# bcgsc/ntJoin

Hardware: AMD Instinct MI355X
Metric: Gbp/s minimizer-sketch+graph-build (k=32,w=1000) (higher is better)
Workload: dtype u64

## Files before the change

ntjoin_amd/csrc/graph.hip:

```cpp
#include <algorithm>
#include <cstdlib>
#include <cstring>
#include <system_error>
#include <thread>

#include "join_verdict.h"
#include "mxg_internal.h"
#include "scan_kernels.h"

namespace mxg {

static constexpr uint64_t HT_EMPTY = 0xFFFFFFFFFFFFFFFFull;
static constexpr uint32_t NONE32 = 0xFFFFFFFFu;

struct Slot {
    unsigned long long key;
    uint32_t nseen, ndup;
};

__device__ __forceinline__ uint32_t ht_slot(Slot *tab, uint32_t mask, uint32_t cap, uint64_t key)
{
    if (key == HT_EMPTY) return cap;
    uint32_t s = (uint32_t)((key * 0x9E3779B97F4A7C15ull) >> 32) & mask;
    while (true) {
        unsigned long long cur = tab[s].key;
        if (cur == key) return s;
        if (cur == HT_EMPTY) {
            unsigned long long old = atomicCAS(&tab[s].key, (unsigned long long)HT_EMPTY, (unsigned long long)key);
            if (old == HT_EMPTY || old == key) return s;
        }
        s = (s + 1) & mask;
    }
}

struct AsmSet {
    uint32_t n_asm;
    uint32_t full;
    uint32_t n[MXG_MAX_ASSEMBLIES];
    const uint32_t *n_ptr[MXG_MAX_ASSEMBLIES];
// ... 852 lines not shown
    const uint32_t rec = p.rec[i];
    p.vpos[v] = p.pos[i];
    p.vrec[v] = rec;
    if (p.ivid) p.ivid[i] = v;
    p.fv[r] = v;
    p.frec[r] = rec;
}

__global__ __launch_bounds__(256) void k_block_prefix(const uint32_t *__restrict__ cnt, const uint32_t *__restrict__ sup, uint32_t n,
                                                      uint32_t *__restrict__ out)
{
    __shared__ uint32_t sh[256];
    __shared__ uint32_t sh_before;
    const uint32_t e = blockIdx.x * 256u + threadIdx.x;
    const uint32_t c = e < n ? cnt[e] : 0u;
    if (threadIdx.x < 64) {
        const uint32_t bef = count_prefix(cnt, sup, blockIdx.x * 256u);
        if (threadIdx.x == 0) sh_before = bef;
    }
    __syncthreads();
    const uint32_t r = sh_before + block_exclusive_256(c, sh);
    if (e < n) out[e] = r;
}

struct VertexPjParams {
    AsmSet as;
    const uint32_t *pos[MXG_MAX_ASSEMBLIES], *rec[MXG_MAX_ASSEMBLIES];
    const uint32_t *cnt, *sup;
    uint64_t *n_shared;
    const uint64_t *mask0;
    const uint32_t *bpref0;
    uint64_t *vhash;
    uint32_t *vpos, *vrec, *fv, *frec;
    uint32_t nvs;
    uint32_t *ivid[MXG_MAX_ASSEMBLIES];
};

template <uint32_t U>
__global__ __launch_bounds__(256) void k_vertices_pj(const VertexPjParams p, uint32_t nb)
{
    __shared__ TailScan<U> ts;
    const uint32_t blk0 = blockIdx.x * U, lane = threadIdx.x & 63u, wv = threadIdx.x >> 6;
    TailAsm t[U];
    tail_asms<U>(p.as, blk0, nb, t);
    uint32_t ia[U], ii[U], vw[U], rec[U], pos[U];
    uint64_t hsh[U];
    bool in[U], f[U];
    {
        uint8_t fl[U];
#pragma unroll
        for (uint32_t u = 0; u < U; ++u) {
            const bool there = blk0 + u < nb;
            const uint32_t a = ia[u] = t[u].a, i = ii[u] = ((there ? blk0 + u : blk0) - t[u].b0) * 256u + threadIdx.x;
            in[u] = there && i < t[u].n;
            const uint32_t ic = in[u] ? i : 0u;
            fl[u] = p.as.flags[a][ic];
            vw[u] = p.as.slot[a][a ? ic : 0u];
            rec[u] = p.rec[a][ic];
            pos[u] = p.pos[a][ic];
            hsh[u] = p.as.hash[0][a ? 0u : ic];
        }
#pragma unroll
        for (uint32_t u = 0; u < U; ++u) f[u] = in[u] & ((fl[u] & MXG_MX_SHARED) != 0);
    }
    uint32_t v0[U];
#pragma unroll
// ... 16 lines not shown
            const uint64_t own = q == 0 ? mlo[g].x : q == 1 ? mlo[g].y : q == 2 ? mhi[g].x : mhi[g].y;
            v0[h + g] = bp[g] + (uint32_t)__popcll(own & ((1ull << (i0 & 63u)) - 1ull)) + (q > 0 ? (uint32_t)__popcll(mlo[g].x) : 0u) +
                        (q > 1 ? (uint32_t)__popcll(mlo[g].y) : 0u) + (q > 2 ? (uint32_t)__popcll(mhi[g].x) : 0u);
        }
        if (U > 2) __builtin_amdgcn_sched_barrier(0);
    }
    uint64_t bm[U];
#pragma unroll
    for (uint32_t u = 0; u < U; ++u) tail_ballot(ts, u, f[u], bm[u]);
    if (wv < U && blk0 + wv < nb) {
        const uint32_t blk_g = blk0 + wv, a = asm_of_block(p.as, blk_g);
        const uint32_t blk = blk_g - p.as.bstart[a], nblk = p.as.bstart[a + 1] - p.as.bstart[a];
        const uint32_t *cnt = p.cnt + p.as.bstart[a], *sup = p.sup + sup_start(p.as, a);
        const uint32_t bef = count_prefix(cnt, sup, blk);
        if (lane == 0) ts.before[wv] = bef;
        if (blk + 1 == nblk) {
            const uint32_t all = count_prefix(cnt, sup, nblk);
            if (lane == 0) p.n_shared[a] = all;
        }
    }
    __syncthreads();
#pragma unroll
    for (uint32_t u = 0; u < U; ++u) {
        if (!in[u]) continue;
        const uint32_t a = ia[u], i = ii[u];
        const uint32_t r = ts.before[u] + tail_rank(ts, u, bm[u]);
        const uint32_t v = a ? v0[u] : r;
        if (p.ivid[a]) p.ivid[a][i] = f[u] ? v : NONE32;
        if (!f[u]) continue;
        if (!a) p.vhash[v] = hsh[u];
        const size_t o = (size_t)a * p.nvs;
        p.vpos[o + v] = pos[u];
        p.vrec[o + v] = rec[u];
        p.fv[o + r] = v;
        p.frec[o + r] = rec[u];
    }
}

template <uint32_t U>
__global__ __launch_bounds__(256) void k_adjacency(const uint32_t *__restrict__ fv0, const uint32_t *__restrict__ frec0,
                                                   const uint64_t *__restrict__ nv_ptr, uint2 *__restrict__ adj0, uint32_t stride)
{
    const size_t o = (size_t)blockIdx.y * stride;
    const uint32_t *fv = fv0 + o, *frec = frec0 + o;
    uint32_t rc[U], rn[U], rp[U], vc[U], vn[U], vp[U];
#pragma unroll
    for (uint32_t u = 0; u < U; ++u) {
        const uint32_t r = (blockIdx.x * U + u) * 256u + threadIdx.x;
        rc[u] = rn[u] = rp[u] = vc[u] = vn[u] = vp[u] = 0;
        if (r < stride) {
            rc[u] = frec[r];
            vc[u] = fv[r];
            if (r + 1 < stride) {
                rn[u] = frec[r + 1];
                vn[u] = fv[r + 1];
            }
            if (r > 0) {
                rp[u] = frec[r - 1];
                vp[u] = fv[r - 1];
            }
        }
    }
    const uint32_t nv = (uint32_t)*nv_ptr;
#pragma unroll
    for (uint32_t u = 0; u < U; ++u) {
        const uint32_t r = (blockIdx.x * U + u) * 256u + threadIdx.x;
        if (r >= nv) continue;
        const uint32_t nx = (r + 1 < nv && rn[u] == rc[u]) ? vn[u] : NONE32;
        const uint32_t pv = (r > 0 && rp[u] == rc[u]) ? vp[u] : NONE32;
        adj0[o + vc[u]] = make_uint2(nx, pv);
    }
}

struct EdgeParams {
    const uint32_t *fv;
    const uint2 *adj;
    const uint64_t *nv_ptr;
    uint32_t nv, n_asm;
    uint8_t *eflag;
    uint32_t *bsum;
    uint32_t *bsuper;
    uint64_t *n_edges;
    uint64_t *host_ctl;
    uint32_t *eu, *ev, *esup;
    double *ew;
    double weights[MXG_MAX_ASSEMBLIES];
};

__device__ __forceinline__ uint32_t edge_mask(const EdgeParams &p, uint32_t u, uint32_t v)
{
    uint32_t m = 0;
    for (uint32_t b = 0; b < p.n_asm; ++b) {
        const uint2 q = p.adj[(size_t)b * p.nv + u];
        if (q.x == v || q.y == v) m |= 1u << b;
    }
    return m;
}

template <uint32_t U>
__global__ __launch_bounds__(256) void k_edge_flags(const EdgeParams p, uint32_t n_items)
{
    __shared__ TailScan<U> ts;
    const uint32_t blk0 = blockIdx.x * U, nblk = (n_items + 255u) / 256u, lane = threadIdx.x & 63u, wv = threadIdx.x >> 6;
    uint32_t uu[U], ia[U];
    bool live[U];
#pragma unroll
    for (uint32_t u = 0; u < U; ++u) {
        const uint32_t item = (blk0 + u) * 256u + threadIdx.x;
        uu[u] = p.fv[blk0 + u < nblk && item < n_items ? item : 0u];
// ... 56 lines not shown
    __shared__ TailScan<U> ts;
    const uint32_t blk0 = blockIdx.x * U, nblk = (n_items + 255u) / 256u, lane = threadIdx.x & 63u, wv = threadIdx.x >> 6;
    uint32_t fb[U], uu[U], v[U], m[U];
#pragma unroll
    for (uint32_t u = 0; u < U; ++u) {
        const uint32_t item = (blk0 + u) * 256u + threadIdx.x;
        const bool in = blk0 + u < nblk && item < n_items;
        fb[u] = p.eflag[in ? item : 0u];
        uu[u] = p.fv[in ? item : 0u];
        if (!in) fb[u] = 0;
    }
#pragma unroll
    for (uint32_t u = 0; u < U; ++u)
        v[u] = p.adj[fb[u] ? (size_t)(((blk0 + u) * 256u + threadIdx.x) / p.nv) * p.nv + uu[u] : (size_t)0].x;
    uint64_t bm[U];
#pragma unroll
    for (uint32_t u = 0; u < U; ++u) tail_ballot(ts, u, fb[u] != 0, bm[u]);
    if (wv < U && blk0 + wv < nblk) {
        const uint32_t bef = count_prefix(p.bsum, p.bsuper, blk0 + wv);
        if (lane == 0) ts.before[wv] = bef;
        if (blk0 + wv + 1 == nblk) {
            const uint32_t all = count_prefix(p.bsum, p.bsuper, nblk);
            if (lane == 0) {
                *p.n_edges = all;
                p.host_ctl[32] = all;
            }
            if (lane < p.n_asm) p.host_ctl[lane] = p.nv_ptr[lane];
        }
    }
#pragma unroll
    for (uint32_t u = 0; u < U; ++u) {
        m[u] = fb[u];
        if (fb[u] && p.n_asm > 8u) m[u] = edge_mask(p, uu[u], v[u]);
    }
    __syncthreads();
#pragma unroll
    for (uint32_t u = 0; u < U; ++u) {
        if (!fb[u]) continue;
        double wsum = 0.0;
        for (uint32_t b = 0; b < p.n_asm; ++b)
            if (m[u] & (1u << b)) wsum = wsum + p.weights[b];
        const uint32_t e = ts.before[u] + tail_rank(ts, u, bm[u]);
        p.eu[e] = uu[u];
        p.ev[e] = v[u];
        p.esup[e] = m[u];
        p.ew[e] = wsum;
    }
}

__global__ __launch_bounds__(256) void k_apply_msgs(const uint4 *__restrict__ msgs, uint64_t n, uint32_t stride, uint32_t *adj)
{
    const uint64_t i = (uint64_t)blockIdx.x * 256u + threadIdx.x;
    if (i >= n) return;
    const uint4 m = msgs[i];
    adj[((size_t)(m.x & 255u) * stride + m.y) * 2u + ((m.x >> 8) ? 1u : 0u)] = m.z;
}

__global__ __launch_bounds__(256) void k_iota_rows(uint32_t *a, uint32_t stride)
{
    const uint32_t i = blockIdx.x * 256u + threadIdx.x;
    if (i < stride) a[(size_t)blockIdx.y * stride + i] = i;
}

template <class T>
static int d2h(mxg_handle *h, std::vector<T> &dst, const void *src, size_t n)
{
// ... 51 lines not shown
    uint32_t pj_force_fail = 0;
    uint64_t *pj_mask0 = nullptr;
    uint32_t *pj_bpref0 = nullptr;
    AsmSet as_all;
    uint32_t n_fsup = 0, n_esup = 0;
    uint32_t *fsup = nullptr, *esup = nullptr, *cnt = nullptr;
    uint32_t *M = nullptr, *cursor = nullptr;
    uint4 *recs1 = nullptr, *recs2 = nullptr;
    PjSubCaps sc;
    size_t clear_words = 0;
};

static int plan_join(mxg_handle *h, int mode, const GraphBounds *gb, bool global_table, bool split, JoinPlan &pl)
{
    const uint32_t A = (uint32_t)h->asms.size();
    if (A == 0) return set_err(h, MXG_EINVAL, "mxg_build_graph: no assemblies");
    if (A > MXG_MAX_ASSEMBLIES) return set_err(h, MXG_ELIMIT, "at most %d assemblies", MXG_MAX_ASSEMBLIES);
    pl = JoinPlan();
    JoinRequest rq;
    rq.A = A;
    for (uint32_t ai = 0; ai < A; ++ai) {
        Assembly *a = h->asms[ai];
        if (!gb && !a->has_sketch) return set_err(h, MXG_EINVAL, "assembly '%s' has no sketch (call mxg_sketch)", a->name.c_str());
        rq.n_of[ai] = gb ? gb->n_bound[ai] : a->n_mx;
    }
    rq.mode = mode;
    rq.bounds = gb != nullptr;
    rq.global_table = global_table;
    rq.split = split;
    const char *join_env = knob_raw(h, "MXG_GRAPH_JOIN");
    rq.join_global = join_env && !strcmp(join_env, "global");
    rq.force_two_level = knob_u64(h, "MXG_PJ_TWO_LEVEL", 0) != 0;
    rq.graph_u = (uint32_t)std::min<uint64_t>(knob_u64(h, "MXG_GRAPH_U", 0), 8);
    rq.pj_tiles = (uint32_t)std::min<uint64_t>(knob_u64(h, "MXG_PJ_TILES", 0), 8);
    rq.no_rec12 = knob_u64(h, "MXG_PJ_REC12", 1) == 0;
    rq.no_pipe = knob_u64(h, "MXG_PJ_PIPE", 1024) == 0;
    rq.no_prefill0 = knob_u64(h, "MXG_PJ_PREFILL0", 1) == 0;
    if (knob_u64(h, "MXG_PJ_SPLIT", 0) && mode == GRAPH_FULL) rq.split = true;
    switch (join_shape(rq, h->pj_learnt, pl)) {
    case JS_TOO_MANY_MINIMIZERS: return set_err(h, MXG_ELIMIT, "too many minimizers for one table (%llu)", (unsigned long long)pl.N);
    case JS_TOO_MANY_ITEMS: return set_err(h, MXG_ELIMIT, "graph too large for 32-bit item indices");
    case JS_OK: break;
    }
    pl.pj_force_fail = knob_u64(h, "MXG_PJ_FORCE_FAIL", 0) ? 1u : 0u;
    pl.sc.n_sub = pl.n_sub;
    for (uint32_t a = 0; a < MXG_MAX_ASSEMBLIES; ++a) pl.sc.cap[a] = pl.sub_cap[a];
    const uint64_t *const n_of = pl.n_of;
    const uint32_t nb = pl.nb, P = pl.P, P1 = pl.P1;

    if (!pl.pj) MXG_HIP(h, h->g_keys.ensure(((size_t)pl.cap + 1) * sizeof(Slot)));
    const size_t nb0 = pl.nb0, nb_all = nb;
    MXG_HIP(h, h->g_vid.ensure(pl.pj ? (nb0 + nb_all) * 4 * 8 + nb0 * 4 + 64 : ((size_t)pl.cap + 1) * 4));
    pl.pj_mask0 = h->g_vid.as<uint64_t>();
    uint64_t *const pj_fol = pl.pj_mask0 + nb0 * 4;
    pl.pj_bpref0 = reinterpret_cast<uint32_t *>(pj_fol + nb_all * 4);
    MXG_HIP(h, h->g_ctl.ensure(CTL_WORDS * 8));

    AsmSet &as_all = pl.as_all;
    as_all.n_asm = A;
    as_all.full = pl.full;
    as_all.fol = pl.pj ? pj_fol : nullptr;
    for (uint32_t a = 0; a < A; ++a) {
        Assembly *as = h->asms[a];
        MXG_HIP(h, as->d_slot.ensure(std::max<uint64_t>(n_of[a] * 4, 16)));
        MXG_HIP(h, as->d_flags.ensure(std::max<uint64_t>(n_of[a], 16)));
        as_all.n[a] = (uint32_t)n_of[a];
// ... 104 lines not shown
    if (fine) MXG_HIP(h, hipEventRecord(e1, st));
    ++h->pj_early_done;
    return MXG_OK;
}

void graph_drop_plan(mxg_handle *h)
{
    delete h->pj_plan;
    h->pj_plan = nullptr;
}

static int take_or_make_plan(mxg_handle *h, const GraphCall &c, bool global_table, JoinPlan &own, const JoinPlan **plan)
{
    const JoinPlan *ep = h->pj_plan;
    bool early = ep && ep->split && h->pj_early_done != 0 && h->pj_early_done == ep->A && c.gb && c.mode == GRAPH_FULL && !global_table &&
                 ep->A == h->asms.size();
    for (uint32_t a = 0; early && a < ep->A; ++a) early = c.gb->n_bound[a] == ep->n_of[a] && c.gb->n_ptr[a] == ep->as_all.n_ptr[a];
    h->pj_early_done = 0;
    *plan = early ? ep : &own;
    if (early) return MXG_OK;
    const int rc = plan_join(h, c.mode, c.gb, global_table, false, own);
    if (rc != MXG_OK && c.mode != GRAPH_DG_EDGES && c.mode != GRAPH_DG_EDGES_APPLIED)
        for (Assembly *a : h->asms) a->flags_valid = a->flags_on_host = false;
    return rc;
}

#define TAIL_LAUNCH(kernel, U, grid, stream, ...)                                                      \
    do {                                                                                               \
        if ((U) == 4) hipLaunchKernelGGL(kernel<4>, grid, dim3(256), 0, stream, __VA_ARGS__);          \
        else if ((U) == 2) hipLaunchKernelGGL(kernel<2>, grid, dim3(256), 0, stream, __VA_ARGS__);     \
        else hipLaunchKernelGGL(kernel<1>, grid, dim3(256), 0, stream, __VA_ARGS__);                   \
    } while (0)

struct GraphStage {
    mxg_handle *const h;
    const GraphCall &c;
    const JoinPlan &pl;
    const bool early;
    const bool resume;
    const bool fine, timing;
    Graph &g;
    uint64_t *ctl = nullptr, *hctl = nullptr;
    uint64_t *pj_fail = nullptr;

    GraphStage(mxg_handle *h_, const GraphCall &c_, const JoinPlan &pl_, bool early_)
        : h(h_), c(c_), pl(pl_), early(early_), resume(c_.mode == GRAPH_DG_EDGES || c_.mode == GRAPH_DG_EDGES_APPLIED),
          fine((h_->cfg.flags & MXG_FLAG_TIMING_FINE) != 0 && c_.mode == GRAPH_FULL), timing((h_->cfg.flags & MXG_FLAG_TIMING) != 0 || fine),
          g(h_->graph)
    {
    }
    bool joins() const { return pl.nb && !resume; }
    size_t anv() const { return (size_t)pl.A * pl.nvs; }

    int begin()
    {
        for (uint32_t ai = 0; ai < pl.A; ++ai) {
            Assembly *a = h->asms[ai];
            if (!resume) a->flags_on_host = false;
            a->flags_valid = true;
        }
        if (!resume) g = Graph();
        g.n_asm = pl.A;
        if (fine && !h->ev_g[0]) {
            MXG_HIP(h, hipEventCreate(&h->ev_g[0]));
            MXG_HIP(h, hipEventCreate(&h->ev_g[1]));
        }
        if (timing) MXG_HIP(h, hipEventRecord(h->ev0, h->stream));
        if (!resume)
            h->stat_graph_join = (pl.pj ? (pl.two_level ? MXG_JOIN_LDS_TWO_LEVEL : MXG_JOIN_LDS) : MXG_JOIN_GLOBAL) | (early ? MXG_JOIN_EARLY : 0);
        if (!resume && knob_u64(h, "MXG_DEBUG_JOIN", 0)) {
            uint32_t t1 = 0;
            for (uint32_t a = 0; pl.pj && pl.two_level && a < (pl.split ? pl.A : 1u); ++a)
                t1 = std::max(t1, pj1_launch_tiles(pl, pl.split ? a : 0u, pl.split ? a + 1 : pl.A));
            fprintf(stderr, "[mxg] join pj=%d two_level=%d split=%d early=%d record_bytes=%d prefill0=%u P1=%u rows2=%u tiles1=%u\n", (int)pl.pj,
                    (int)pl.two_level, (int)pl.split, (int)early, pl.rec12 ? 12 : 16, pl.prefill0, pl.P1, pl.rows2, t1);
        }
        if (!pl.pj && !resume) MXG_HIP(h, hipMemsetAsync(h->g_keys.p, 0xFF, ((size_t)pl.cap + 1) * sizeof(Slot), h->stream));
        ctl = h->g_ctl.as<uint64_t>();
        if (!h->pinned_gctl) MXG_HIP(h, hipHostMalloc((void **)&h->pinned_gctl, CTL_WORDS * 8));
        hctl = h->pinned_gctl;
        memset(hctl, 0, CTL_WORDS * 8);
        pj_fail = pl.dg_pj ? dg_pj_fail_word(h) : hctl + CTL_PJ_FAIL;
        return MXG_OK;
    }

    void launch_join(uint4 *recs, uint32_t *M, uint32_t n_parts, uint32_t n_rows, const uint32_t *cursor)
    {
        const bool narrow = pl.A <= 16;
        const uint32_t cap1 = cursor ? pl.cap1 : 0u, rows2 = cursor ? pl.rows2 : 0u;
        const uint64_t pipe_blocks = cursor ? knob_u64(h, "MXG_PJ_PIPE", 1024) : 0;
        const uint32_t prefill0 = cursor ? pl.prefill0 : 0u;
        if (pipe_blocks && rows2 <= 256) {
            auto kernel = pl.rec12 ? (narrow ? k_pj_join_pipe<true, true> : k_pj_join_pipe<false, true>)
                                   : (narrow ? k_pj_join_pipe<true, false> : k_pj_join_pipe<false, false>);
            hipLaunchKernelGGL(kernel, dim3((uint32_t)std::min<uint64_t>(pipe_blocks, n_parts)), dim3(256), 0, h->stream, recs, M, pl.P, n_parts,
                               pj_fail, pl.pj_force_fail, cursor, cap1, rows2, pl.as_all, pl.sc, prefill0);
        } else
            hipLaunchKernelGGL(narrow ? k_pj_join<true> : k_pj_join<false>, dim3(n_parts), dim3(256), 0, h->stream, recs, M, pl.P, n_rows,
                               pj_fail, pl.pj_force_fail, cursor, cap1, rows2, pl.as_all, pl.sc, prefill0);
    }
    void flags_pj()
    {
        TAIL_LAUNCH(k_flags_pj, pl.u_flags, dim3(graph_tail_grid(pl.nb, pl.u_flags)), h->stream, pl.as_all, pl.nb, pl.cnt, pl.fsup, pl.pj_mask0);
    }
    int join_two_level()
    {
        if (!early && pl.split) {
            MXG_HIP(h, hipMemsetAsync(pl.fsup, 0, pl.clear_words * 4, h->stream));
// ... 42 lines not shown
        MXG_HIP(h, h->g_frec.ensure(anv() * 4));
        MXG_HIP(h, h->g_nxt.ensure(2 * anv() * 4));
        if (c.mode == GRAPH_DG_EDGES) MXG_HIP(h, hipMemsetAsync(h->g_nxt.p, 0xFF, 2 * anv() * 4, h->stream));
        return MXG_OK;
    }
    int item_vids(uint32_t a, uint32_t **ivid)
    {
        *ivid = nullptr;
        if (c.mode != GRAPH_DG_VERTICES) return MXG_OK;
        MXG_HIP(h, h->asms[a]->d_ivid.ensure((size_t)pl.n_of[a] * 4 + 16));
        *ivid = h->asms[a]->d_ivid.as<uint32_t>();
        return MXG_OK;
    }
    int fill(VertexPjParams &vp)
    {
        vp.as = pl.as_all;
        for (uint32_t a = 0; a < MXG_MAX_ASSEMBLIES; ++a) {
            vp.pos[a] = a < pl.A ? h->asms[a]->d_pos.as<uint32_t>() : nullptr;
            vp.rec[a] = a < pl.A ? h->asms[a]->d_rec.as<uint32_t>() : nullptr;
            vp.ivid[a] = nullptr;
            int rc;
            if (a < pl.A && (rc = item_vids(a, &vp.ivid[a])) != MXG_OK) return rc;
        }
        vp.cnt = pl.cnt;
        vp.sup = pl.fsup;
        vp.n_shared = ctl + CTL_SHARED;
        vp.mask0 = pl.pj_mask0;
        vp.bpref0 = pl.pj_bpref0;
        vp.vhash = h->g_vhash.as<uint64_t>();
        vp.vpos = h->g_vpos.as<uint32_t>();
        vp.vrec = h->g_vrec.as<uint32_t>();
        vp.fv = h->g_fv.as<uint32_t>();
        vp.frec = h->g_frec.as<uint32_t>();
        vp.nvs = (uint32_t)pl.nvs;
        return MXG_OK;
    }
    int vertices_pj()
    {
        VertexPjParams vp;
        const int rc = fill(vp);
        if (rc != MXG_OK) return rc;
        hipLaunchKernelGGL(k_block_prefix, dim3((uint32_t)((pl.nb0 + 255) / 256)), dim3(256), 0, h->stream, pl.cnt + pl.as_all.bstart[0],
                           pl.fsup + sup_start(pl.as_all, 0), (uint32_t)pl.nb0, pl.pj_bpref0);
        TAIL_LAUNCH(k_vertices_pj, pl.u_vertices, dim3(graph_tail_grid(pl.nb, pl.u_vertices)), h->stream, vp, pl.nb);
        return MXG_OK;
    }
    int fill(VertexParams &vp, uint32_t a)
    {
        Assembly *as = h->asms[a];
        const size_t row = (size_t)a * pl.nvs;
        vp.flags = as->d_flags.as<uint8_t>();
        vp.cnt = pl.cnt + pl.as_all.bstart[a];
        vp.sup = pl.fsup + sup_start(pl.as_all, a);
        vp.n_shared = ctl + CTL_SHARED + a;
        vp.slot = as->d_slot.as<uint32_t>();
        vp.hash = as->d_hash.as<uint64_t>();
        vp.pos = as->d_pos.as<uint32_t>();
        vp.rec = as->d_rec.as<uint32_t>();
        vp.n = (uint32_t)pl.n_of[a];
        vp.n_ptr = c.gb ? c.gb->n_ptr[a] : nullptr;
        vp.first = a == 0;
        vp.vid = h->g_vid.as<uint32_t>();
        vp.vhash = h->g_vhash.as<uint64_t>();
        vp.vpos = h->g_vpos.as<uint32_t>() + row;
        vp.vrec = h->g_vrec.as<uint32_t>() + row;
        vp.fv = h->g_fv.as<uint32_t>() + row;
// ... 8 lines not shown
            if (rc != MXG_OK) return rc;
            if (vp.ivid) MXG_HIP(h, hipMemsetAsync(vp.ivid, 0xFF, (size_t)vp.n * 4, h->stream));
            hipLaunchKernelGGL(k_vertices, dim3((vp.n + 255) / 256), dim3(256), 0, h->stream, vp);
        }
        return MXG_OK;
    }
    int hand_back_vertices()
    {
        g.nv_stride = pl.nvs;
        if (!c.d_n_vertices) return MXG_OK;
        if (pl.nvs > 0) MXG_HIP(h, hipMemcpyAsync(c.d_n_vertices, ctl + CTL_SHARED, 8, hipMemcpyDeviceToDevice, h->stream));
        else MXG_HIP(h, hipMemsetAsync(c.d_n_vertices, 0, 8, h->stream));
        return MXG_OK;
    }

    void adjacency_own()
    {
        TAIL_LAUNCH(k_adjacency, pl.u_edges, dim3(graph_tail_grid((pl.nvs + 255) / 256, pl.u_edges), pl.A), h->stream, h->g_fv.as<uint32_t>(),
                    h->g_frec.as<uint32_t>(), ctl + CTL_SHARED, h->g_nxt.as<uint2>(), (uint32_t)pl.nvs);
    }
    void adjacency_of_owner()
    {
        if (c.n_msgs && c.mode == GRAPH_DG_EDGES)
            hipLaunchKernelGGL(k_apply_msgs, dim3((uint32_t)((c.n_msgs + 255) / 256)), dim3(256), 0, h->stream,
                               static_cast<const uint4 *>(c.d_msgs), c.n_msgs, (uint32_t)pl.nvs, h->g_nxt.as<uint32_t>());
        hipLaunchKernelGGL(k_iota_rows, dim3((uint32_t)((pl.nvs + 255) / 256), pl.A), dim3(256), 0, h->stream, h->g_fv.as<uint32_t>(),
                           (uint32_t)pl.nvs);
    }

    void fill(EdgeParams &ep)
    {
        ep.fv = h->g_fv.as<uint32_t>();
        ep.adj = h->g_nxt.as<uint2>();
        ep.nv_ptr = ctl + CTL_SHARED;
        ep.nv = (uint32_t)pl.nvs;
        ep.n_asm = pl.A;
        ep.eflag = h->g_eflag.as<uint8_t>();
        ep.bsum = h->g_ebs.as<uint32_t>();
        ep.bsuper = pl.esup;
        ep.n_edges = ctl + CTL_EDGES;
        ep.host_ctl = hctl;
        ep.eu = h->g_eu.as<uint32_t>();
        ep.ev = h->g_ev.as<uint32_t>();
        ep.esup = h->g_esup.as<uint32_t>();
        ep.ew = h->g_ew.as<double>();
        for (uint32_t a = 0; a < MXG_MAX_ASSEMBLIES; ++a) ep.weights[a] = a < pl.A ? h->asms[a]->weight : 0.0;
    }
    int edges()
    {
        const uint32_t n_items = pl.n_items;
        MXG_HIP(h, h->g_eflag.ensure(n_items));
        MXG_HIP(h, h->g_ebs.ensure((size_t)pl.e_blocks * 4 + 64));
        MXG_HIP(h, h->g_eu.ensure((size_t)n_items * 4));
        MXG_HIP(h, h->g_ev.ensure((size_t)n_items * 4));
        MXG_HIP(h, h->g_esup.ensure((size_t)n_items * 4));
        MXG_HIP(h, h->g_ew.ensure((size_t)n_items * 8));
        EdgeParams ep;
        fill(ep);
        const dim3 grid(graph_tail_grid(pl.e_blocks, pl.u_edges));
        TAIL_LAUNCH(k_edge_flags, pl.u_edges, grid, h->stream, ep, n_items);
        TAIL_LAUNCH(k_edges, pl.u_edges, grid, h->stream, ep, n_items);
        MXG_HIP(h, hipGetLastError());
        return MXG_OK;
    }

    int sync_and_verdict()
    {
        if (timing) MXG_HIP(h, hipEventRecord(h->ev1, h->stream));
        MXG_HIP(h, stream_wait(h->stream));
        if (!pl.pj || !hctl[CTL_PJ_FAIL]) return MXG_OK;
        if (!pl.two_level || pl.pj_force_fail) return RC_RETRY_GLOBAL;
        std::vector<uint32_t> cur((size_t)pl.P1 * pl.n_sub * PJ1_CS);
        MXG_HIP(h, hipMemcpy(cur.data(), pl.cursor, cur.size() * 4, hipMemcpyDeviceToHost));
        return join_overflow_verdict(pl, cur.data(), h->pj_learnt);
    }
    int results()
    {
        const uint64_t nv = hctl[CTL_SHARED];
        for (uint32_t a = 1; a < pl.A; ++a)
            if (hctl[CTL_SHARED + a] != nv)
                return set_err(h, MXG_EDEVICE, "internal error: shared-minimizer counts differ between assemblies (%llu vs %llu)",
                               (unsigned long long)hctl[CTL_SHARED + a], (unsigned long long)nv);
        g.nv = nv;
        if (c.mode == GRAPH_FULL) h->pj_learnt.shared_counted(pl.pre_sig, nv, pl.n_of[0]);
        g.nv_stride = pl.nvs;
        g.ne = pl.nvs > 0 ? hctl[CTL_EDGES] : 0;
        h->stat_unique = ~0ull;
        if (timing) {
            float ms = 0;
            MXG_HIP(h, hipEventElapsedTime(&ms, h->ev0, h->ev1));
            h->tm.ms_graph += ms;
            if (fine && pl.nvs > 0) {
                float a = 0, b = 0, c3 = 0;
                MXG_HIP(h, hipEventElapsedTime(&a, h->ev0, h->ev_g[0]));
                MXG_HIP(h, hipEventElapsedTime(&b, h->ev_g[0], h->ev_g[1]));
                MXG_HIP(h, hipEventElapsedTime(&c3, h->ev_g[1], h->ev1));
                h->tm.ms_join += a;
                h->tm.ms_vertices += b;
                h->tm.ms_edges += c3;
            }
        }
        g.valid = true;
        g.own_order = c.mode == GRAPH_FULL;
        g.host_valid = false;
        return MXG_OK;
    }
};

static int build_graph_impl(mxg_handle *h, const GraphCall &c, bool global_table)
{
    MXG_HIP(h, hipSetDevice(h->device));
    JoinPlan own;
    const JoinPlan *plan = nullptr;
    int rc = take_or_make_plan(h, c, global_table, own, &plan);
    if (rc != MXG_OK) return rc;
    const JoinPlan &pl = *plan;
    GraphStage s(h, c, pl, plan != &own);
    if ((rc = s.begin()) != MXG_OK) return rc;
    if (s.joins() && (rc = pl.pj ? (pl.two_level ? s.join_two_level() : s.join_one_level()) : s.join_global()) != MXG_OK) return rc;
    if ((rc = s.mark(h->ev_g[0])) != MXG_OK) return rc;
    if (pl.nvs > 0) {
        if ((rc = s.vertex_arrays()) != MXG_OK) return rc;
        if (!s.resume && (rc = pl.pj ? s.vertices_pj() : s.vertices_global()) != MXG_OK) return rc;
    }
    if (c.mode == GRAPH_DG_VERTICES) return s.hand_back_vertices();
    if (pl.nvs > 0) {
        if (c.mode == GRAPH_FULL) s.adjacency_own();
        else s.adjacency_of_owner();
        if ((rc = s.mark(h->ev_g[1])) != MXG_OK) return rc;
        if ((rc = s.edges()) != MXG_OK) return rc;
    }
    if ((rc = s.sync_and_verdict()) != MXG_OK) return rc;
    return s.results();
}

int graph_to_host(mxg_handle *h)
{
    Graph &g = h->graph;
    if (!g.valid) return set_err(h, MXG_EINVAL, "call mxg_build_graph first");
    if (g.host_valid) return MXG_OK;
    MXG_HIP(h, hipSetDevice(h->device));
    const size_t anv = (size_t)g.n_asm * g.nv;
    int rc;
    {
        std::vector<std::thread> th;
        auto sized = [](auto &v, size_t n) {
            try {
                v.resize(n);
            } catch (const std::bad_alloc &) {
            }
        };
        try {
            th.emplace_back([&] { sized(g.vhash, g.nv); });
            th.emplace_back([&] { sized(g.vpos, anv); });
            th.emplace_back([&] { sized(g.vrec, anv); });
            th.emplace_back([&] { sized(g.eu, g.ne); });
            th.emplace_back([&] { sized(g.ev, g.ne); });
            th.emplace_back([&] { sized(g.esup, g.ne); });
            sized(g.ew, g.ne);
        } catch (const std::system_error &) {
        }
// ... 34 lines not shown
```

ntjoin_amd/csrc/join_plan.h:

```cpp
#pragma once
#include <algorithm>
#include <cstddef>
#include <cstdint>

#include "ntjoin_mx.h"

#if defined(__HIPCC__)
#define PJP_HD __host__ __device__ inline
#else
#define PJP_HD inline
#endif

namespace mxg {

enum { GRAPH_FULL = 0, GRAPH_DG_VERTICES = 1, GRAPH_DG_EDGES = 2, GRAPH_DG_EDGES_APPLIED = 3  };

constexpr uint32_t PJ_IPB = 4096;
constexpr uint32_t PJ_T = 2048;
constexpr uint32_t PJ_MAX_P = 4096;
constexpr uint32_t PJ1_CS = 32;
constexpr uint32_t PJ_CAP_LIMIT = 0xFFFFF000u;

struct JoinLearnt {
    bool overflowed = false;
// ... 69 lines not shown
    return (((1u << f) - 1u) << PJ12_FINE_SHIFT) | (((1u << (PJ12_TAG_BITS - f)) - 1u) << PJ12_COARSE_SHIFT);
}
PJP_HD uint32_t pj12_tag(uint32_t assembly, bool dup) { return assembly | (dup ? PJ12_TAG_DUP : 0u); }
PJP_HD uint32_t pj12_pack(uint32_t prod_hi, uint32_t lgP, uint32_t tag)
{
    const uint32_t f = pj12_fine_bits(lgP);
    return (prod_hi & ~pj12_tag_mask(lgP)) | ((tag & ((1u << f) - 1u)) << PJ12_FINE_SHIFT) | ((tag >> f) << PJ12_COARSE_SHIFT);
}
PJP_HD uint32_t pj12_unpack_tag(uint32_t word, uint32_t lgP)
{
    const uint32_t f = pj12_fine_bits(lgP);
    return ((word >> PJ12_FINE_SHIFT) & ((1u << f) - 1u)) | (((word >> PJ12_COARSE_SHIFT) & ((1u << (PJ12_TAG_BITS - f)) - 1u)) << f);
}
PJP_HD uint64_t pj12_key(uint32_t lo, uint32_t word, uint32_t lgP) { return ((uint64_t)(word & ~pj12_tag_mask(lgP)) << 32) | lo; }
PJP_HD bool pj12_same_key(uint32_t lo_a, uint32_t word_a, uint32_t lo_b, uint32_t word_b, uint32_t lgP)
{
    return pj12_key(lo_a, word_a, lgP) == pj12_key(lo_b, word_b, lgP);
}
PJP_HD uint32_t pj12_coarse(uint64_t prod, uint32_t P1) { return (uint32_t)(prod >> 52) & (P1 - 1u); }
PJP_HD uint32_t pj12_fine(uint64_t prod, uint32_t P) { return (uint32_t)(prod >> 44) & (P - 1u); }

struct JoinRequest {
    uint32_t A = 0;
    uint64_t n_of[MXG_MAX_ASSEMBLIES] = {};
    int mode = GRAPH_FULL;
    bool bounds = false;
    bool global_table = false;
    bool split = false;
    bool force_two_level = false;
    bool join_global = false;
    bool no_rec12 = false;
    bool no_pipe = false;
    bool no_prefill0 = false;
    uint32_t graph_u = 0;
    uint32_t pj_tiles = 0;
};

enum JoinShapeError { JS_OK = 0, JS_TOO_MANY_MINIMIZERS, JS_TOO_MANY_ITEMS };

struct JoinShape {
    uint32_t A = 0;
    uint64_t N = 0, nvs = 0;
    uint64_t n_of[MXG_MAX_ASSEMBLIES] = {};
    uint32_t cap = 0, mask = 0, full = 0;
    uint32_t P = 0, P1 = 0, cap1 = 0, rows2 = 0;
    bool two_level = false, pj = false, dg_pj = false;
    bool split = false;
    uint32_t n_sub = 1;
    uint32_t sub_cap[MXG_MAX_ASSEMBLIES] = {}, sub_off[MXG_MAX_ASSEMBLIES] = {}, skew_lim[MXG_MAX_ASSEMBLIES] = {};
    uint32_t bstart[MXG_MAX_ASSEMBLIES + 1] = {};
    uint32_t nb = 0;
    size_t nb0 = 0;
    uint32_t n_items = 0, e_blocks = 0;
    bool rec12 = false;
    uint32_t prefill0 = 0;
    uint64_t pre_sig = 0;
    size_t n_cur = 0;
    uint32_t u_flags = 1, u_vertices = 1, u_edges = 1;
    uint32_t pj_tiles_forced = 0;
};

constexpr uint32_t GRAPH_TAIL_U2 = 3072, GRAPH_TAIL_U4 = 8192;
constexpr uint32_t GRAPH_TAIL_U_VERTICES = 2;
inline uint32_t graph_tail_u(uint64_t blocks, uint32_t forced = 0)
{
    if (forced == 1 || forced == 2 || forced == 4) return forced;
    return blocks >= GRAPH_TAIL_U4 ? 4u : blocks >= GRAPH_TAIL_U2 ? 2u : 1u;
}
inline uint32_t graph_tail_grid(uint64_t blocks, uint32_t U) { return (uint32_t)((blocks + U - 1) / U); }

constexpr uint32_t PJ1_TILES_G2 = 0xFFFFFFFFu;

inline uint32_t pj1_tiles(uint64_t tiles, bool rec12, uint32_t forced = 0)
{
    if (!rec12) return 1u;
    if (forced == 1 || forced == 2) return forced;
    return tiles >= PJ1_TILES_G2 ? 2u : 1u;
}
inline uint32_t pj_tiles_grid(uint64_t tiles, uint32_t G) { return (uint32_t)((tiles + G - 1) / G); }

inline JoinShapeError join_shape(const JoinRequest &rq, const JoinLearnt &learnt, JoinShape &pl)
{
    pl = JoinShape();
    const uint32_t A = pl.A = rq.A;
    uint64_t N = 0, nmin = ~0ull, n_max = 0;
    for (uint32_t a = 0; a < A; ++a) {
        pl.n_of[a] = rq.n_of[a];
        N += rq.n_of[a];
        nmin = std::min(nmin, rq.n_of[a]);
        n_max = std::max(n_max, rq.n_of[a]);
    }
// ... 29 lines not shown
            fits32 = c_all <= PJ_CAP_LIMIT;
        } else {
            uint64_t c1 = (N / P1) + (N / P1) / 4 + 4096;
            if (learnt.cap1_P1 == P1) c1 = std::max<uint64_t>(c1, learnt.cap1_need);
            cap1 = (uint32_t)((c1 + PJ_IPB - 1) / PJ_IPB * PJ_IPB);
            pl.sub_cap[0] = cap1;
        }
        pl.rows2 = cap1 / PJ_IPB;
    }
    pl.P = P;
    pl.P1 = P1;
    pl.cap1 = cap1;
    pl.two_level = P1 != 0 && P1 <= 4096 && fits32 && (uint64_t)P1 * cap1 < (1ull << 32) && (uint64_t)P1 * P * (PJ_T + 1) < (1ull << 29);
    pl.dg_pj = rq.mode == GRAPH_DG_VERTICES && rq.bounds && !learnt.dg_off;
    pl.pj = (rq.mode == GRAPH_FULL || pl.dg_pj) && !rq.global_table && (P1 == 0 || pl.two_level) && P <= PJ_MAX_P && n_max < (1ull << 29) &&
            !rq.join_global;
    for (uint32_t a = 0; a < A; ++a) {
        pl.bstart[a] = pl.nb;
        pl.nb += (uint32_t)((rq.n_of[a] + 255) / 256);
    }
    for (uint32_t a = A; a <= MXG_MAX_ASSEMBLIES; ++a) pl.bstart[a] = pl.nb;
    pl.nb0 = (size_t)((rq.n_of[0] + 255) / 256);
    pl.nvs = nmin;
    if (pl.nvs > 0 && (uint64_t)A * pl.nvs >= (1ull << 32)) return JS_TOO_MANY_ITEMS;
    pl.n_items = (uint32_t)((size_t)A * pl.nvs);
    pl.e_blocks = (pl.n_items + 255) / 256;
    if (pl.split && pl.pj && pl.two_level) pl.n_cur = (size_t)P1 * A * PJ1_CS;
    pl.rec12 = pl.split && pl.pj && pl.two_level && pj12_fits(P1, P) && pl.rows2 <= 256 && !rq.no_rec12 && !rq.no_pipe;
    pl.pre_sig = JoinLearnt::prefill_signature(A, rq.n_of, rq.bounds);
    pl.prefill0 = pl.pj && pl.two_level && !rq.no_prefill0 && learnt.prefill_own0(pl.pre_sig) ? 1u : 0u;
    pl.u_flags = graph_tail_u(pl.nb, rq.graph_u);
    pl.u_vertices = graph_tail_u(0, rq.graph_u) == rq.graph_u ? rq.graph_u : std::min(pl.u_flags, GRAPH_TAIL_U_VERTICES);
    pl.u_edges = graph_tail_u(pl.e_blocks, rq.graph_u);
    pl.pj_tiles_forced = rq.pj_tiles == 1 || rq.pj_tiles == 2 ? rq.pj_tiles : 0u;
    return JS_OK;
}

inline uint32_t pj1_launch_tiles(const JoinShape &pl, uint32_t a_lo, uint32_t a_hi)
{
    const uint32_t tiles = (pl.bstart[a_hi] - pl.bstart[a_lo] + PJ_IPB / 256 - 1) / (PJ_IPB / 256);
    return pj1_tiles(tiles, pl.rec12, pl.pj_tiles_forced);
}

enum JoinRetry { RC_RETRY_GLOBAL = 1, RC_RETRY_PJ = 2 };

inline JoinRetry join_overflow_verdict(const JoinShape &pl, const uint32_t *cur, JoinLearnt &learnt)
{
    const uint32_t P1 = pl.P1, n_sub = pl.n_sub;
    uint64_t mx = 0;
    for (uint32_t c = 0; c < P1; ++c) {
        uint64_t all = 0;
        for (uint32_t s = 0; s < n_sub; ++s) all += cur[((size_t)c * n_sub + s) * PJ1_CS];
        mx = std::max(mx, all);
    }
    if (pl.split) {
        bool grew = false;
        if (learnt.sub_P1 != P1) std::fill_n(learnt.sub_need, MXG_MAX_ASSEMBLIES, 0ull);
        learnt.sub_P1 = P1;
        for (uint32_t s = 0; s < n_sub; ++s) {
            uint64_t ms = 0;
            for (uint32_t c = 0; c < P1; ++c) ms = std::max<uint64_t>(ms, cur[((size_t)c * n_sub + s) * PJ1_CS]);
            if (ms > pl.sub_cap[s] && learnt.sub_need[s] < ms) {
                learnt.sub_need[s] = ms + ms / 8 + 4096;
                grew = true;
            }
        }
// ... 16 lines not shown
```

Before: 2765.

## Derive edge support from per-assembly vertex ranks instead of adjacency table

The vertex kernel now records each vertex's rank within every non-reference assembly. In full-graph mode the adjacency build pass is skipped, and edge support is tested by checking whether two vertices have adjacent ranks in the same record. New rank-based edge-flag and edge-emit kernels are specialised for small assembly counts, with gathers unrolled per assembly, and whole blocks that cover no items exit early. This removes the adjacency kernel and its scattered uint2 writes, in exchange for more random gathers into the rank and record arrays, plus added code complexity.

```diff
diff --git a/ntjoin_amd/csrc/graph.hip b/ntjoin_amd/csrc/graph.hip
--- a/ntjoin_amd/csrc/graph.hip
+++ b/ntjoin_amd/csrc/graph.hip
@@ -5,6 +5,7 @@
 #include <thread>
 
 #include "join_verdict.h"
+#include "graph_rank.h"
 #include "mxg_internal.h"
 #include "scan_kernels.h"
 
@@ -923,6 +924,7 @@
     const uint32_t *bpref0;
     uint64_t *vhash;
     uint32_t *vpos, *vrec, *fv, *frec;
+    uint32_t *rank;
     uint32_t nvs;
     uint32_t *ivid[MXG_MAX_ASSEMBLIES];
 };
@@ -1005,6 +1007,7 @@
         const size_t o = (size_t)a * p.nvs;
         p.vpos[o + v] = pos[u];
         p.vrec[o + v] = rec[u];
+        if (a && p.rank) p.rank[o + v] = r;
         p.fv[o + r] = v;
         p.frec[o + r] = rec[u];
     }
@@ -1048,6 +1051,7 @@
 struct EdgeParams {
     const uint32_t *fv;
     const uint2 *adj;
+    const uint32_t *frec, *rank;
     const uint64_t *nv_ptr;
     uint32_t nv, n_asm;
     uint8_t *eflag;
@@ -1170,6 +1174,166 @@
     for (uint32_t u = 0; u < U; ++u) {
         m[u] = fb[u];
         if (fb[u] && p.n_asm > 8u) m[u] = edge_mask(p, uu[u], v[u]);
+    }
+    __syncthreads();
+#pragma unroll
+    for (uint32_t u = 0; u < U; ++u) {
+        if (!fb[u]) continue;
+        double wsum = 0.0;
+        for (uint32_t b = 0; b < p.n_asm; ++b)
+            if (m[u] & (1u << b)) wsum = wsum + p.weights[b];
+        const uint32_t e = ts.before[u] + tail_rank(ts, u, bm[u]);
+        p.eu[e] = uu[u];
+        p.ev[e] = v[u];
+        p.esup[e] = m[u];
+        p.ew[e] = wsum;
+    }
+}
+
+__device__ __forceinline__ uint32_t edge_mask_rank(const EdgeParams &p, uint32_t u, uint32_t v)
+{
+    const uint32_t last = p.nv - 1u;
+    return rank_support_mask(
+        p.n_asm, u, v, [&](uint32_t b, uint32_t x) { return b ? p.rank[(size_t)b * p.nv + min(x, last)] : x; },
+        [&](uint32_t b, uint32_t r) { return p.frec[(size_t)b * p.nv + min(r, last)]; });
+}
+
+template <uint32_t U, uint32_t NB>
+__global__ __launch_bounds__(256) void k_edge_flags_rank(const EdgeParams p, uint32_t n_items)
+{
+    __shared__ TailScan<U> ts;
+    const uint32_t blk0 = blockIdx.x * U, nblk = (n_items + 255u) / 256u, lane = threadIdx.x & 63u, wv = threadIdx.x >> 6;
+    constexpr uint32_t K = NB ? NB : 1u;
+    const uint32_t nvc = (uint32_t)*p.nv_ptr;
+    if (rank_items_unused(blk0 * 256u, U * 256u, n_items, p.nv, nvc)) {
+        if (wv < U && lane == 0 && blk0 + wv < nblk) count_publish(p.bsum, p.bsuper, blk0 + wv, 0u);
+        return;
+    }
+    uint32_t uu[U], vv[U], rc[U], rn[U], r0[U][K], r1[U][K];
+    bool in[U];
+#pragma unroll
+    for (uint32_t u = 0; u < U; ++u) {
+        const uint32_t item = (blk0 + u) * 256u + threadIdx.x;
+        in[u] = blk0 + u < nblk && item < n_items;
+        const uint32_t i0 = in[u] ? item : 0u, i1 = in[u] && item + 1u < n_items ? item + 1u : 0u;
+        const bool first = item < p.nv;
+        uu[u] = p.fv[first ? 0u : i0];
+        vv[u] = p.fv[first ? 0u : i1];
+        if (first) uu[u] = item, vv[u] = item + 1u;
+        rc[u] = p.frec[i0];
+        rn[u] = p.frec[i1];
+        const uint32_t j0 = in[u] && first ? item : 0u, j1 = in[u] && item + 1u < p.nv ? item + 1u : 0u;
+#pragma unroll
+        for (uint32_t k = 0; k < NB; ++k) {
+            const size_t row = k + 1u < p.n_asm ? (size_t)(k + 1u) * p.nv : (size_t)0;
+            r0[u][k] = p.rank[row + j0];
+            r1[u][k] = p.rank[row + j1];
+        }
+    }
+    uint32_t ia[U];
+    bool succ[U];
+#pragma unroll
+    for (uint32_t u = 0; u < U; ++u) {
+        const uint32_t item = (blk0 + u) * 256u + threadIdx.x;
+        ia[u] = in[u] ? item / p.nv : 0u;
+        succ[u] = in[u] && item - ia[u] * p.nv + 1u < nvc && rn[u] == rc[u];
+    }
+    uint8_t f[U];
+    if constexpr (NB > 0) {
+        uint32_t gu[U][K], gv[U][K];
+#pragma unroll
+        for (uint32_t u = 0; u < U; ++u)
+#pragma unroll
+            for (uint32_t k = 1; k < NB; ++k) {
+                const uint32_t b = k < ia[u] ? k : k + 1u;
+                const bool need = succ[u] && ia[u] != 0u && b < p.n_asm && uu[u] < p.nv && vv[u] < p.nv;
+                const size_t row = need ? (size_t)b * p.nv : (size_t)0;
+                gu[u][k] = p.rank[row + (need ? uu[u] : 0u)];
+                gv[u][k] = p.rank[row + (need ? vv[u] : 0u)];
+            }
+        uint32_t x[U][K], y[U][K];
+        bool w[U][K];
+#pragma unroll
+        for (uint32_t u = 0; u < U; ++u)
+#pragma unroll
+            for (uint32_t k = 0; k < NB; ++k) {
+                const uint32_t b = k < ia[u] ? k : k + 1u;
+                const uint32_t ru = ia[u] == 0u ? r0[u][k] : k == 0u ? uu[u] : gu[u][k];
+                const uint32_t rv = ia[u] == 0u ? r1[u][k] : k == 0u ? vv[u] : gv[u][k];
+                uint32_t lo, hi;
+                w[u][k] = rank_fetch(succ[u] && b < p.n_asm, ru, rv, p.nv, lo, hi);
+                const size_t row = w[u][k] ? (size_t)b * p.nv : (size_t)0;
+                x[u][k] = p.frec[row + lo];
+                y[u][k] = p.frec[row + hi];
+            }
+#pragma unroll
+        for (uint32_t u = 0; u < U; ++u) {
+            uint32_t m = 1u << ia[u];
+#pragma unroll
+            for (uint32_t k = 0; k < NB; ++k)
+                if (w[u][k] && x[u][k] == y[u][k]) m |= 1u << (k < ia[u] ? k : k + 1u);
+            f[u] = succ[u] ? rank_edge_flag(m, ia[u], p.n_asm) : (uint8_t)0;
+        }
+    } else {
+#pragma unroll
+        for (uint32_t u = 0; u < U; ++u) {
+            f[u] = 0;
+            if (!succ[u]) continue;
+            f[u] = rank_edge_flag(edge_mask_rank(p, uu[u], vv[u]), ia[u], p.n_asm);
+        }
+    }
+#pragma unroll
+    for (uint32_t u = 0; u < U; ++u) {
+        const uint32_t item = (blk0 + u) * 256u + threadIdx.x;
+        if (in[u]) p.eflag[item] = f[u];
+        uint64_t bm;
+        tail_ballot(ts, u, f[u] != 0, bm);
+    }
+    __syncthreads();
+    if (wv < U && lane == 0 && blk0 + wv < nblk) count_publish(p.bsum, p.bsuper, blk0 + wv, tail_total(ts, wv));
+}
+
+template <uint32_t U>
+__global__ __launch_bounds__(256) void k_edges_rank(const EdgeParams p, uint32_t n_items)
+{
+    __shared__ TailScan<U> ts;
+    const uint32_t blk0 = blockIdx.x * U, nblk = (n_items + 255u) / 256u, lane = threadIdx.x & 63u, wv = threadIdx.x >> 6;
+    auto report_totals = [&]() {
+        const uint32_t all = count_prefix(p.bsum, p.bsuper, nblk);
+        if (lane == 0) {
+            *p.n_edges = all;
+            p.host_ctl[32] = all;
+        }
+        if (lane < p.n_asm) p.host_ctl[lane] = p.nv_ptr[lane];
+    };
+    if (rank_items_unused(blk0 * 256u, U * 256u, n_items, p.nv, (uint32_t)*p.nv_ptr)) {
+        if (wv < U && blk0 + wv + 1 == nblk) report_totals();
+        return;
+    }
+    uint32_t fb[U], uu[U], v[U], m[U];
+#pragma unroll
+    for (uint32_t u = 0; u < U; ++u) {
+        const uint32_t item = (blk0 + u) * 256u + threadIdx.x;
+        const bool in = blk0 + u < nblk && item < n_items;
+        const bool first = item < p.nv;
+        fb[u] = p.eflag[in ? item : 0u];
+        uu[u] = p.fv[in && !first ? item : 0u];
+        v[u] = p.fv[in && !first && item + 1u < n_items ? item + 1u : 0u];
+        if (first) uu[u] = item, v[u] = item + 1u;
+        if (!in) fb[u] = 0;
+    }
+    uint64_t bm[U];
+#pragma unroll
+    for (uint32_t u = 0; u < U; ++u) tail_ballot(ts, u, fb[u] != 0, bm[u]);
+    if (wv < U && blk0 + wv < nblk) {
+        const uint32_t bef = count_prefix(p.bsum, p.bsuper, blk0 + wv);
+        if (lane == 0) ts.before[wv] = bef;
+        if (blk0 + wv + 1 == nblk) report_totals();
+    }
+#pragma unroll
+    for (uint32_t u = 0; u < U; ++u) {
+        m[u] = fb[u];
+        if (fb[u] && p.n_asm > 8u) m[u] = edge_mask_rank(p, uu[u], v[u]);
     }
     __syncthreads();
 #pragma unroll
@@ -1287,6 +1451,7 @@
     rq.join_global = join_env && !strcmp(join_env, "global");
     rq.force_two_level = knob_u64(h, "MXG_PJ_TWO_LEVEL", 0) != 0;
     rq.graph_u = (uint32_t)std::min<uint64_t>(knob_u64(h, "MXG_GRAPH_U", 0), 8);
+    rq.no_graph_rank = knob_u64(h, "MXG_GRAPH_RANK", 1) == 0;
     rq.pj_tiles = (uint32_t)std::min<uint64_t>(knob_u64(h, "MXG_PJ_TILES", 0), 8);
     rq.no_rec12 = knob_u64(h, "MXG_PJ_REC12", 1) == 0;
     rq.no_pipe = knob_u64(h, "MXG_PJ_PIPE", 1024) == 0;
@@ -1457,6 +1622,13 @@
         else hipLaunchKernelGGL(kernel<1>, grid, dim3(256), 0, stream, __VA_ARGS__);                   \
     } while (0)
 
+#define TAIL_LAUNCH2(kernel, U, X, grid, stream, ...)                                                  \
+    do {                                                                                               \
+        if ((U) == 4) hipLaunchKernelGGL((kernel<4, X>), grid, dim3(256), 0, stream, __VA_ARGS__);     \
+        else if ((U) == 2) hipLaunchKernelGGL((kernel<2, X>), grid, dim3(256), 0, stream, __VA_ARGS__); \
+        else hipLaunchKernelGGL((kernel<1, X>), grid, dim3(256), 0, stream, __VA_ARGS__);              \
+    } while (0)
+
 struct GraphStage {
     mxg_handle *const h;
     const GraphCall &c;
@@ -1497,8 +1669,8 @@
             uint32_t t1 = 0;
             for (uint32_t a = 0; pl.pj && pl.two_level && a < (pl.split ? pl.A : 1u); ++a)
                 t1 = std::max(t1, pj1_launch_tiles(pl, pl.split ? a : 0u, pl.split ? a + 1 : pl.A));
-            fprintf(stderr, "[mxg] join pj=%d two_level=%d split=%d early=%d record_bytes=%d prefill0=%u P1=%u rows2=%u tiles1=%u\n", (int)pl.pj,
-                    (int)pl.two_level, (int)pl.split, (int)early, pl.rec12 ? 12 : 16, pl.prefill0, pl.P1, pl.rows2, t1);
+            fprintf(stderr, "[mxg] join pj=%d two_level=%d split=%d early=%d record_bytes=%d prefill0=%u P1=%u rows2=%u tiles1=%u rank=%d\n",
+                    (int)pl.pj, (int)pl.two_level, (int)pl.split, (int)early, pl.rec12 ? 12 : 16, pl.prefill0, pl.P1, pl.rows2, t1, (int)pl.graph_rank);
         }
         if (!pl.pj && !resume) MXG_HIP(h, hipMemsetAsync(h->g_keys.p, 0xFF, ((size_t)pl.cap + 1) * sizeof(Slot), h->stream));
         ctl = h->g_ctl.as<uint64_t>();
@@ -1607,6 +1779,7 @@
         vp.vrec = h->g_vrec.as<uint32_t>();
         vp.fv = h->g_fv.as<uint32_t>();
         vp.frec = h->g_frec.as<uint32_t>();
+        vp.rank = pl.graph_rank ? h->g_nxt.as<uint32_t>() : nullptr;
         vp.nvs = (uint32_t)pl.nvs;
         return MXG_OK;
     }
@@ -1681,6 +1854,8 @@
     {
         ep.fv = h->g_fv.as<uint32_t>();
         ep.adj = h->g_nxt.as<uint2>();
+        ep.frec = h->g_frec.as<uint32_t>();
+        ep.rank = h->g_nxt.as<uint32_t>();
         ep.nv_ptr = ctl + CTL_SHARED;
         ep.nv = (uint32_t)pl.nvs;
         ep.n_asm = pl.A;
@@ -1707,8 +1882,15 @@
         EdgeParams ep;
         fill(ep);
         const dim3 grid(graph_tail_grid(pl.e_blocks, pl.u_edges));
-        TAIL_LAUNCH(k_edge_flags, pl.u_edges, grid, h->stream, ep, n_items);
-        TAIL_LAUNCH(k_edges, pl.u_edges, grid, h->stream, ep, n_items);
+        if (pl.graph_rank) {
+            if (pl.A <= 2) TAIL_LAUNCH2(k_edge_flags_rank, pl.u_edges, 1, grid, h->stream, ep, n_items);
+            else if (pl.A <= 4) TAIL_LAUNCH2(k_edge_flags_rank, pl.u_edges, 3, grid, h->stream, ep, n_items);
+            else TAIL_LAUNCH2(k_edge_flags_rank, pl.u_edges, 0, grid, h->stream, ep, n_items);
+            TAIL_LAUNCH(k_edges_rank, pl.u_edges, grid, h->stream, ep, n_items);
+        } else {
+            TAIL_LAUNCH(k_edge_flags, pl.u_edges, grid, h->stream, ep, n_items);
+            TAIL_LAUNCH(k_edges, pl.u_edges, grid, h->stream, ep, n_items);
+        }
         MXG_HIP(h, hipGetLastError());
         return MXG_OK;
     }
@@ -1774,8 +1956,8 @@
     }
     if (c.mode == GRAPH_DG_VERTICES) return s.hand_back_vertices();
     if (pl.nvs > 0) {
-        if (c.mode == GRAPH_FULL) s.adjacency_own();
-        else s.adjacency_of_owner();
+        if (c.mode != GRAPH_FULL) s.adjacency_of_owner();
+        else if (!pl.graph_rank) s.adjacency_own();
         if ((rc = s.mark(h->ev_g[1])) != MXG_OK) return rc;
         if ((rc = s.edges()) != MXG_OK) return rc;
     }
diff --git a/ntjoin_amd/csrc/graph_rank.h b/ntjoin_amd/csrc/graph_rank.h
--- /dev/null
+++ b/ntjoin_amd/csrc/graph_rank.h
@@ -0,0 +1,51 @@
+#pragma once
+#include <cstdint>
+
+#if defined(__HIPCC__) || defined(__CUDACC__)
+#define GRK_HD __host__ __device__ inline
+#else
+#define GRK_HD inline
+#endif
+
+namespace mxg {
+
+GRK_HD bool rank_adjacent(uint32_t ru, uint32_t rv) { return ru + 1u == rv || rv + 1u == ru; }
+
+GRK_HD bool rank_neighbours(uint32_t ru, uint32_t rv, uint32_t rec_u, uint32_t rec_v) { return rank_adjacent(ru, rv) && rec_u == rec_v; }
+
+GRK_HD bool rank_fetch(bool wanted, uint32_t ru, uint32_t rv, uint32_t stride, uint32_t &lo, uint32_t &hi)
+{
+    const bool f = wanted && rank_adjacent(ru, rv) && ru < stride && rv < stride;
+    lo = f ? (ru < rv ? ru : rv) : 0u;
+    hi = f ? (ru < rv ? rv : ru) : 0u;
+    return f;
+}
+
+GRK_HD bool rank_items_unused(uint32_t first, uint32_t n, uint32_t n_items, uint32_t stride, uint32_t count)
+{
+    if (first >= n_items || n == 0u || count == 0u) return true;
+    const uint32_t last = (uint32_t)((uint64_t)first + n <= n_items ? first + n - 1u : n_items - 1u);
+    const uint32_t a = first / stride;
+    return first - a * stride >= count && last / stride == a;
+}
+
+template <class RankOf, class RecAt>
+GRK_HD uint32_t rank_support_mask(uint32_t n_asm, uint32_t u, uint32_t v, RankOf rank_of, RecAt rec_at)
+{
+    uint32_t m = 0;
+    for (uint32_t b = 0; b < n_asm; ++b) {
+        const uint32_t ru = rank_of(b, u), rv = rank_of(b, v);
+        if (rank_adjacent(ru, rv) && rec_at(b, ru) == rec_at(b, rv)) m |= 1u << b;
+    }
+    return m;
+}
+
+GRK_HD bool rank_first_supporter(uint32_t mask, uint32_t a) { return mask != 0u && (uint32_t)__builtin_ctz(mask) == a; }
+
+GRK_HD uint8_t rank_edge_flag(uint32_t mask, uint32_t a, uint32_t n_asm)
+{
+    if (!rank_first_supporter(mask, a)) return 0;
+    return n_asm <= 8u ? (uint8_t)mask : (uint8_t)1;
+}
+
+}
diff --git a/ntjoin_amd/csrc/join_plan.h b/ntjoin_amd/csrc/join_plan.h
--- a/ntjoin_amd/csrc/join_plan.h
+++ b/ntjoin_amd/csrc/join_plan.h
@@ -125,6 +125,7 @@
     bool no_rec12 = false;
     bool no_pipe = false;
     bool no_prefill0 = false;
+    bool no_graph_rank = false;
     uint32_t graph_u = 0;
     uint32_t pj_tiles = 0;
 };
@@ -150,6 +151,7 @@
     uint64_t pre_sig = 0;
     size_t n_cur = 0;
     uint32_t u_flags = 1, u_vertices = 1, u_edges = 1;
+    bool graph_rank = false;
     uint32_t pj_tiles_forced = 0;
 };
 
@@ -245,6 +247,7 @@
     pl.u_flags = graph_tail_u(pl.nb, rq.graph_u);
     pl.u_vertices = graph_tail_u(0, rq.graph_u) == rq.graph_u ? rq.graph_u : std::min(pl.u_flags, GRAPH_TAIL_U_VERTICES);
     pl.u_edges = graph_tail_u(pl.e_blocks, rq.graph_u);
+    pl.graph_rank = rq.mode == GRAPH_FULL && pl.pj && !rq.no_graph_rank;
     pl.pj_tiles_forced = rq.pj_tiles == 1 || rq.pj_tiles == 2 ? rq.pj_tiles : 0u;
     return JS_OK;
 }
```

New measurement: 2846 (median of 6 runs). 2.9% higher.
